# nomic-ai/contrastors

Hardware: AMD Instinct MI355X
Metric: query-doc pairs/sec (whole node), nomic-bert-2048 seq128 global-batch 16384 (higher is better)
Workload: dtype bf16

## Files before the change

### contrastors_amd/_C.py

```python
from __future__ import annotations

import ctypes as C
import os
from pathlib import Path

_PKG = Path(__file__).resolve().parent
LIB_PATH = Path(os.environ.get("CONTRASTORS_HIP_LIB", _PKG / "lib" / "libcontrastors_hip.so"))

CX_OK = 0
_ERR = {-1: "CX_ERR_SHAPE", -2: "CX_ERR_ALIGN", -3: "CX_ERR_ARG", -4: "CX_ERR_LAUNCH"}

vp = C.c_void_p
i32 = C.c_int
i64 = C.c_long
f32 = C.c_float
u64 = C.c_ulonglong
u32 = C.c_uint


class CxLayerWeights(C.Structure):
    _fields_ = (
        [(n, vp) for n in ("Wqkv", "Wout", "Wfc1", "Wfc2", "WqkvT", "WoutT", "Wfc1T", "Wfc2T")]
        + [(n, vp) for n in ("bqkv", "bout", "bfc1", "bfc2")]
        + [(n, vp) for n in ("ln1_g", "ln1_b", "ln2_g", "ln2_b")]
# ... 41 lines not shown


class CxVitExt(C.Structure):
    _fields_ = [("rope_cos", vp), ("rope_sin", vp), ("n_rope", i32), ("n_prefix", i32), ("no_final_ln", i32),
                ("subln_eps", f32), ("sub_ln", C.POINTER(CxVitSubLN)), ("z", vp), ("zmean", vp), ("zrstd", vp),
                ("yg_wide", vp)]


_SIGS = {
    "cx_abi_version": (i32, []),
    "cx_build_info": (C.c_char_p, []),
    "cx_error_string": (C.c_char_p, [i32]),
    "cx_gemm_bf16_nt": (i32, [vp, vp, vp, vp, i32, i32, i32, i32, i32, i32, i32, i32, f32, vp]),
    "cx_gemm_bf16_nt_accum": (i32, [vp, vp, vp, vp, i64, i32, i32, i32, i32, i32, vp]),
    "cx_gemm_bf16_tn_accum": (i32, [vp, vp, vp, vp, i64, i32, i32, i32, i32, i32, vp]),
    "cx_prof_gemm_config": (i32, [i32, i32]),
    "cx_prof_gemm_collect": (i32, [C.POINTER(C.c_double), C.POINTER(C.c_double), C.POINTER(i64), C.POINTER(i64)]),
    "cx_calib_mfma_bf16": (i32, [vp, i32, i32, vp, vp, vp]),
    "cx_calib_copy": (i32, [vp, vp, i64, vp]),
    "cx_transpose_bf16": (i32, [vp, vp, i32, i32, i32, i32, i32, vp]),
    "cx_cast_f32_to_bf16": (i32, [vp, vp, i64, vp]),
    "cx_cast_transpose_f32_to_bf16": (i32, [vp, vp, i32, i32, vp]),
    "cx_cast_transpose_f32_to_bf16_batched": (i32, [vp, i32, i32, vp]),
    "cx_cast_bf16_to_f32": (i32, [vp, vp, i64, vp]),
    "cx_layernorm_fwd": (i32, [vp, vp, vp, vp, vp, vp, vp, vp, i32, i32, f32, vp]),
    "cx_layernorm_bwd": (i32, [vp, vp, vp, vp, vp, vp, vp, vp, vp, vp, vp, i64, i32, i32, vp]),
    "cx_layernorm_bwd_pooled": (i32, [vp, vp, vp, vp, i32, i32, i32, vp, vp, vp, vp, vp, vp, vp, vp, vp, i64, i32, i32, vp]),
    "cx_layernorm_bwd_colsum": (i32, [vp, vp, vp, vp, vp, vp, vp, vp, vp, vp, vp, vp, i64, i32, i32, vp]),
    "cx_dropout_add_layernorm_fwd": (i32, [vp, vp, vp, vp, vp, vp, vp, vp, i32, i32, f32, f32, C.c_ulonglong, C.c_ulonglong,
                                           C.c_uint, vp]),
# ... 126 lines not shown
}

_DEV_SIGS = {
    "cx_gemm_set_variant": (None, [i32]),
    "cx_gemm_get_variant": (i32, []),
    "cx_gemm_set_debug": (None, [i32]),
    "cx_gemm_set_trace": (None, [vp]),
    "cx_gemm_v6_ablate": (None, [i32]),
    "cx_gemm_v6_trace": (None, [vp]),
    "cx_gemm_v7_mode": (None, [i32]),
    "cx_gemm_v7_trace": (None, [vp]),
    "cx_gemm_v7_occupancy": (i32, []),
    "cx_gemm_v7_ablate": (None, [i32]),
    "cx_gemm_v7_flags": (None, [i32]),
    "cx_gemm_v7_period": (None, [i32]),
    "cx_gemm_set_glds": (None, [i32]),
    "cx_gemm_get_glds": (i32, []),
    "cx_attn_set_bwd_s128": (None, [i32]),
    "cx_attn_set_prio": (None, [i32]),
    "cx_attn_set_fwd_s128": (None, [i32]),
    "cx_attn_set_fwd_long": (None, [i32]),
    "cx_attn_set_bwd_long": (None, [i32]),
    "cx_probe_mfma_layout": (i32, [vp, vp]),
    "cx_probe_ds_read_tr16": (i32, [vp, vp, vp]),
    "cx_probe_mfma_rate": (i32, [vp, i32, i32, i32, vp, vp, vp]),
    "cx_attn_dropout_keep_mask": (i32, [vp, i32, i32, i32, f32, u64, u64, u32, vp]),
    "cx_probe_rmw": (i32, [vp, i64, i32, i32, i32, vp]),
    "cx_probe_mfma_rate16": (i32, [vp, i32, i32, i32, vp, vp, vp]),
    "cx_probe_dma_bw": (i32, [vp, i64, i64, i64, i32, i32, i32, i32, vp, vp]),
}
# ... 58 lines not shown
```

### contrastors_amd/csrc/engine.hip

```cpp
#include <hip/hip_runtime.h>
#include "../../include/contrastors_hip.h"
#include "ln_workspace.h"

namespace {

#define CX_TRY(expr)              \
    do {                          \
        int rc__ = (expr);        \
        if (rc__ != CX_OK) return rc__; \
    } while (0)

inline long round_up(long v, long m) { return (v + m - 1) / m * m; }

inline int mark_grads_done(const CxChunkBuffers* buf, int idx, void* stream) {
    if (!buf->layer_events || !buf->layer_events[idx]) return CX_OK;
    return hipEventRecord((hipEvent_t)buf->layer_events[idx], (hipStream_t)stream) == hipSuccess ? CX_OK : CX_ERR_LAUNCH;
}

struct Slots {
    const CxChunkBuffers* b;
    const CxEncoderDesc* e;
    long T_cap;
    int d, I, wfc1;
    int mode;
// ... 58 lines not shown
    return (int)s;
}

int wgrad(const uint16_t* dY, int out_f, const uint16_t* X, int in_f, float* gW, const CxChunkBuffers* b, int T,
          void* stream) {
    if (!gW) return CX_OK;
    const int rc = cx_gemm_bf16_tn_accum(dY, X, gW, b->ws_f32, b->ws_floats, T, out_f, in_f, out_f, in_f, stream);
    if (rc != CX_ERR_SHAPE) return rc;
    if (!b->tr_a || !b->tr_b) return CX_ERR_ARG;
    const int Tp = (int)round_up(T, 64);
    CX_TRY(cx_transpose_bf16(dY, b->tr_a, T, out_f, out_f, Tp, Tp, stream));
    CX_TRY(cx_transpose_bf16(X, b->tr_b, T, in_f, in_f, Tp, Tp, stream));
    return cx_gemm_bf16_nt_accum(b->tr_a, b->tr_b, gW, b->ws_f32, b->ws_floats, out_f, in_f, Tp, Tp, Tp, stream);
}

int proj_residual(const uint16_t* x, const uint16_t* W, const float* bias, const uint16_t* residual, uint16_t* out, int T,
                  int N, int K, bool* folded, void* stream, const CxChunkBuffers* buf = nullptr) {
    *folded = false;
    if (buf && buf->ws_f32 && (long)((T + 255) / 256) * ((N + 255) / 256) <= 64 && K >= 1536) {
        const int rc = cx_gemm_bf16_nt_splitk(x, W, out, bias, residual, buf->ws_f32, buf->ws_floats, T, N, K, K, K, N, N, stream);
        if (rc != CX_ERR_SHAPE) {
            *folded = residual != nullptr && rc == CX_OK;
            return rc;
        }
    }
    if (residual) {
        const int rc = cx_gemm_bf16_nt_residual(x, W, out, bias, residual, T, N, K, K, K, N, N, stream);
        if (rc != CX_ERR_SHAPE) {
            *folded = rc == CX_OK;
            return rc;
// ... 174 lines not shown
};

int blocks_backward(const CxEncoderDesc* enc, const CxChunkBuffers* buf, const Slots& s, const int32_t* cu_seqlens, int Bc,
                    int T, int max_seqlen, const PooledGrad* pg, const uint16_t** da_out, const uint16_t** db_out, void* stream,
                    const CxVitExt* ext = nullptr) {
    const int d = enc->d, I = enc->d_inner, H = enc->n_head, L = enc->n_layer;
    auto mlp_bwd = [&](const CxLayerWeights& w, int l, const uint16_t* dm, const uint16_t* mlp_in, const uint16_t* add,
                       bool* folded, bool bias_done) -> int {
        if (w.gbfc2 && !bias_done) CX_TRY(cx_bias_grad(dm, w.gbfc2, T, d, d, stream));
        if (ext_subln(ext)) {
            CX_TRY(wgrad(dm, d, s.ez(ext, l), I, w.gWfc2, buf, T, stream));
            CX_TRY(cx_gemm_bf16_nt(dm, w.Wfc2T, buf->g_act, nullptr, T, I, d, d, d, I, 0, 1, 1.f, stream));
            const CxVitSubLN& n = ext->sub_ln[l];
            CX_TRY(cx_swiglu_subln_bwd(buf->g_act, s.act(l), s.yg(l), s.ezmean(ext, l), s.ezrstd(ext, l), n.norm_g, buf->g_wide,
                                       n.gnorm_g, n.gnorm_b, w.gbfc1, buf->ws_f32, buf->ws_floats, T, I, stream));
            CX_TRY(wgrad(buf->g_wide, s.wfc1, mlp_in, d, w.gWfc1, buf, T, stream));
            return proj_residual(buf->g_wide, w.Wfc1T, nullptr, add, buf->g_b, T, d, s.wfc1, folded, stream, buf);
        }
        CX_TRY(wgrad(dm, d, s.act(l), I, w.gWfc2, buf, T, stream));
        int fused = CX_ERR_SHAPE;
        if (enc->gated)
            fused = cx_gemm_bf16_swiglu_bwd_gate(dm, w.Wfc2T, s.act(l), s.yg(l), buf->g_wide, T, I, d, d, d, I, s.wfc1, stream);
#ifndef CX_AB_R5_ROUTES
        if (!enc->gated && gelu_fused_shape(T, s.wfc1, d))
            fused = cx_gemm_bf16_act_bwd(dm, w.Wfc2T, s.yg(l), buf->g_wide, w.gbfc1, buf->ws_f32, buf->ws_floats, T, I, d, d, d, I, I,
                                         enc->mlp_act, stream);
#endif
        if (fused != CX_ERR_SHAPE) {
            CX_TRY(fused);
        } else {
            CX_TRY(cx_gemm_bf16_nt(dm, w.Wfc2T, buf->g_act, nullptr, T, I, d, d, d, I, 0, 1, 1.f, stream));
        }
        if (enc->gated) {
            if (fused == CX_ERR_SHAPE)
                CX_TRY(cx_swiglu_bwd_gate(buf->g_act, s.act(l), s.yg(l), buf->g_wide, T, I, stream));
        } else if (fused == CX_ERR_SHAPE) {
            CX_TRY(cx_bias_act_bwd_colsum(buf->g_act, s.yg(l), gelu_fused_shape(T, s.wfc1, d) ? nullptr : w.bfc1, buf->g_wide,
                                          w.gbfc1, T, I, enc->mlp_act, stream));
        }
        CX_TRY(wgrad(buf->g_wide, s.wfc1, mlp_in, d, w.gWfc1, buf, T, stream));
        return proj_residual(buf->g_wide, w.Wfc1T, nullptr, add, buf->g_b, T, d, s.wfc1, folded, stream, buf);
    };
    auto attn_bwd = [&](const CxLayerWeights& w, int l, const uint16_t* dx, const uint16_t* attn_in, const uint16_t* add,
                        bool* folded, bool bias_done) -> int {
        if (w.gbout && !bias_done) CX_TRY(cx_bias_grad(dx, w.gbout, T, d, d, stream));
        CX_TRY(wgrad(dx, d, s.ctx(l), d, w.gWout, buf, T, stream));
        CX_TRY(cx_gemm_bf16_nt(dx, w.WoutT, buf->g_b, nullptr, T, d, d, d, d, d, 0, 1, 1.f, stream));
        if (buf->drop_active && enc->attn_pdrop > 0.f) {
            CX_TRY(cx_attn_varlen_dropout_bwd(buf->g_b, s.qkv(l), s.ctx(l), s.lse(l), cu_seqlens, enc->rot_cos, enc->rot_sin,
                                              buf->delta, buf->g_wide, Bc, H, T, max_seqlen, enc->softmax_scale, enc->attn_pdrop,
                                              buf->drop_seed, buf->drop_offset, (unsigned)(2 * enc->n_layer + 1 + l), stream));
        } else if (enc->rot_cos && max_seqlen > 128) {
            CX_TRY(cx_attn_varlen_bwd_prerotated(buf->g_b, s.qkv(l), s.ctx(l), s.lse(l), cu_seqlens, enc->rot_cos, enc->rot_sin,
                                                 buf->delta, buf->g_wide, Bc, H, T, max_seqlen, enc->softmax_scale, stream));
        } else {
            CX_TRY(cx_attn_varlen_bwd(buf->g_b, s.qkv(l), s.ctx(l), s.lse(l), cu_seqlens, enc->rot_cos, enc->rot_sin,
                                      buf->delta, buf->g_wide, Bc, H, T, max_seqlen, enc->softmax_scale, stream));
        }
        if (ext_rope(ext))
            CX_TRY(cx_rope2d_qkv_inplace(buf->g_wide, cu_seqlens, ext->rope_cos, ext->rope_sin, ext->n_rope, Bc, H, T, ext->n_prefix,
                                         -1, stream));
        if (w.gbqkv) CX_TRY(cx_bias_grad(buf->g_wide, w.gbqkv, T, 3 * d, 3 * d, stream));
        CX_TRY(wgrad(buf->g_wide, 3 * d, attn_in, d, w.gWqkv, buf, T, stream));
        return proj_residual(buf->g_wide, w.WqkvT, nullptr, add, buf->g_b, T, d, 3 * d, folded, stream, buf);
    };
    const bool ws_holds_colsum = cx_ln_bwd_ws_holds(buf->ws_f32, buf->ws_floats, 3, d);
    auto ln_bwd = [&](const uint16_t* a, const uint16_t* b2, const uint16_t* z, const float* g, const float* mean,
                      const float* rstd, const uint16_t* dz_extra, uint16_t* dz, float* gg, float* gb, float* gbias,
                      bool* done) -> int {
        *done = gbias && ws_holds_colsum;
        return cx_layernorm_bwd_colsum(a, b2, z, g, mean, rstd, dz_extra, dz, gg, gb, *done ? gbias : nullptr, buf->ws_f32,
                                       buf->ws_floats, T, d, stream);
    };
    const BlockRunner run{enc, buf, s, cu_seqlens, Bc, T, max_seqlen, stream, ext};
    if (!enc->prenorm) {
        const uint16_t* da = buf->g_a;
        const uint16_t* db = nullptr;
        for (int l = L - 1; l >= 0; --l) {
// ... 398 lines not shown

int cx_abi_version(void) { return 10; }
const char* cx_build_info(void) { return "contrastors_hip gfx950 " __DATE__ " " __VERSION__; }
const char* cx_error_string(int code) {
    switch (code) {
        case CX_OK: return "ok";
        case CX_ERR_SHAPE: return "unsupported shape";
        case CX_ERR_ALIGN: return "misaligned pointer or leading dimension";
        case CX_ERR_ARG: return "invalid argument";
        case CX_ERR_LAUNCH: return "kernel launch failed";
        default: return "unknown error";
    }
}

}
```

### contrastors_amd/csrc/gemm_api.hip

```cpp
#include "cx_common.h"
#include "../../include/contrastors_hip.h"
#include "gemm_params.h"
#include <mutex>

namespace {

constexpr int BK = 64;

__global__ __launch_bounds__(256) void splitk_reduce_kernel(const float* __restrict__ part, float* __restrict__ out, long n4,
                                                            long slab, int splits) {
    const long stride = (long)gridDim.x * blockDim.x;
    for (long i = (long)blockIdx.x * blockDim.x + threadIdx.x; i < n4; i += stride) {
        float4 a = reinterpret_cast<const float4*>(out)[i];
        for (int s = 0; s < splits; ++s) {
            const float4 v = reinterpret_cast<const float4*>(part + s * slab)[i];
            a.x += v.x; a.y += v.y; a.z += v.z; a.w += v.w;
        }
        reinterpret_cast<float4*>(out)[i] = a;
    }
}

int reduce_slabs(const float* ws, float* out, long slab, int split, hipStream_t s) {
    const long n4 = slab / 4;
    long g = (n4 + 255) / 256;
// ... 112 lines not shown
    if (ws_floats < slab) return CX_ERR_SHAPE;
    const int Tp = (T + BK - 1) / BK * BK;
    GemmParams p = base_params(dY, A, ws, nullptr, O, I, Tp, ld_dy, ld_a, I);
    const long tiles = (long)(O / 256) * (I / 256), nk = Tp / BK;
    long max_split = nk / 4;
    if (max_split > ws_floats / slab) max_split = ws_floats / slab;
    if (max_split > 32) max_split = 32;
    p.split_k = (int)choose_split(tiles, max_split);
    {
        ProfScope prof(2.0 * (double)T * (double)O * (double)I, (hipStream_t)stream);
        if (cx_launch_gemm_v6_tn(p, (hipStream_t)stream) != hipSuccess) return CX_ERR_LAUNCH;
    }
    return reduce_slabs(ws, G, slab, p.split_k, (hipStream_t)stream);
}

int cx_gemm_bf16_swiglu(const uint16_t* X, const uint16_t* W, uint16_t* YG, uint16_t* Act, int M, int I, int K, int ldx,
                        int ldw, int ld_yg, int ld_act, void* stream) {
    if (M <= 0 || I <= 0) return CX_OK;
    if (K <= 0 || (K % BK) != 0 || (I % 32) != 0) return CX_ERR_SHAPE;
    if ((ldx % 8) != 0 || (ldw % 8) != 0 || (ld_yg % 4) != 0 || (ld_act % 4) != 0) return CX_ERR_ALIGN;
    if (!Act) return CX_ERR_ARG;
    GemmParams p = base_params(X, W, YG, nullptr, M, 2 * I, K, ldx, ldw, ld_yg);
    p.Out2 = Act; p.ldo2 = ld_act;
    ProfScope prof(2.0 * (double)M * (double)(2 * I) * (double)K, (hipStream_t)stream);
    const hipError_t e = ((ld_yg % 8) == 0 && (ld_act % 8) == 0)
                             ? cx_launch_gemm_v6(p, GEMM_EPI_SWIGLU, (hipStream_t)stream)
                             : cx_launch_gemm_v5(p, 0, GEMM_OUT_BF16, GEMM_EPI_SWIGLU, (hipStream_t)stream);
    return e == hipSuccess ? CX_OK : CX_ERR_LAUNCH;
}

// ... 118 lines not shown
```

### contrastors_amd/csrc/gemm_bf16.hip

```cpp
#include "cx_common.h"
#include "../../include/contrastors_hip.h"
#include "gemm_params.h"

namespace {

constexpr int BM = 128, BN = 128, BK = 64;
constexpr int TILE_BYTES = 128 * BK * 2;

typedef __attribute__((address_space(3))) void* lds_void_ptr;
typedef const __attribute__((address_space(1))) void* glb_void_ptr;

enum OutMode { OUT_BF16 = GEMM_OUT_BF16, OUT_F32 = GEMM_OUT_F32, OUT_F32_ATOMIC = GEMM_OUT_F32_ATOMIC };

struct StageRegs { uint4 r0, r1, r2, r3; };

CX_DEVICE uint4 stage_load(const bf16_t* __restrict__ base, int ld, int row0, int nrows, int k0, int tid, int p) {
    const int r = p * 32 + (tid >> 3);
    int gr = row0 + r;
    gr = gr < nrows ? gr : nrows - 1;
    return *reinterpret_cast<const uint4*>(base + (size_t)gr * ld + k0 + (tid & 7) * 8);
}

template <bool GLDS>
CX_DEVICE void stage_tile(const bf16_t* __restrict__ base, int ld, int row0, int nrows, int k0, char* lds_tile,
// ... 721 lines not shown
    if (use_v5) {
        if (cx_launch_gemm_v5(p, 1, GEMM_OUT_F32_PARTIAL, GEMM_EPI_NONE, (hipStream_t)stream) != hipSuccess) return CX_ERR_LAUNCH;
    } else {
        hipLaunchKernelGGL(gemm_bf16_tn_kernel, dim3((int)(tiles * split)), dim3(512), V2_NSTAGE * V2_STAGE,
                           (hipStream_t)stream, p);
    }
    if (slot >= 0) (void)hipEventRecord(g_prof.ev1[slot], (hipStream_t)stream);
    if (hipGetLastError() != hipSuccess) return CX_ERR_LAUNCH;
    const long n4 = slab / 4;
    long g = (n4 + 255) / 256;
    if (g > 2048) g = 2048;
    hipLaunchKernelGGL(splitk_reduce_kernel, dim3((int)g), dim3(256), 0, (hipStream_t)stream, ws, G, n4, slab, (int)split);
    return hipGetLastError() == hipSuccess ? CX_OK : CX_ERR_LAUNCH;
}

int cx_gemm_bf16_swiglu(const uint16_t* X, const uint16_t* W, uint16_t* YG, uint16_t* Act, int M, int I, int K, int ldx,
                        int ldw, int ld_yg, int ld_act, void* stream) {
    if (M <= 0 || I <= 0) return CX_OK;
    if (K <= 0 || (K % BK) != 0 || (I % 32) != 0) return CX_ERR_SHAPE;
    if ((ldx % 8) != 0 || (ldw % 8) != 0 || (ld_yg % 4) != 0 || (ld_act % 4) != 0) return CX_ERR_ALIGN;
    if (!Act) return CX_ERR_ARG;
    GemmParams p;
    p.X = X; p.W = W; p.Out = YG; p.bias = nullptr;
    p.M = M; p.N = 2 * I; p.K = K; p.ldx = ldx; p.ldw = ldw; p.ldo = ld_yg;
    p.tiles_m = p.tiles_n = 0; p.split_k = 1; p.alpha = 1.f; p.dbg = g_dbg;
    p.Out2 = Act; p.ldo2 = ld_act; p.sup_m = p.sup_n = 0;
    int slot = -1;
    if (g_prof.enabled) {
        if ((g_prof.launches % g_prof.stride) == 0 && g_prof.used < GemmProf::CAP) {
            slot = g_prof.used++;
// ... 192 lines not shown
```

### contrastors_amd/csrc/gemm_bf16_v6.hip

```cpp
#include "cx_common.h"
#include "../../include/contrastors_hip.h"
#include "gemm_params.h"
#include <type_traits>

namespace {

#ifndef CX_V6_HI_EARLY
#define CX_V6_HI_EARLY 1
#endif
#ifndef CX_V6_OPAQUE
#define CX_V6_OPAQUE 1
#endif
#ifndef CX_V6_NT
#define CX_V6_NT 3
#endif
template <int J>
__device__ __forceinline__ void v6_dma_m0(uint32_t slot_base) {
    asm volatile("s_add_u32 m0, %0, %1" ::"s"(slot_base), "n"(J * 4096) : "memory", "scc");
}
__device__ __forceinline__ void v6_dma_ld(uint32_t off, const bf16_t* base) {
    asm volatile("global_load_lds_dwordx4 %0, %1" ::"v"(off), "s"(base) : "memory");
}
template <int J>
__device__ __forceinline__ void v6_dma_full(uint32_t slot_base, uint32_t off, const bf16_t* base) {
// ... 1117 lines not shown
template <int EPI, int DBG = 0>
hipError_t launch6(const GemmParams& p, hipStream_t stream) {
    static CxLdsOptIn lds;
    if (!lds.ensure(reinterpret_cast<const void*>(&gemm_bf16_v6_kernel<EPI, DBG>), LDS6)) return hipErrorInvalidValue;
    const int ntiles = p.tiles_m * p.tiles_n;
    const int grid = ntiles < 256 ? (ntiles + 7) / 8 * 8 : 256;
    hipLaunchKernelGGL((gemm_bf16_v6_kernel<EPI, DBG>), dim3(grid), dim3(256), LDS6, stream, p);
    return hipGetLastError();
}

typedef __attribute__((address_space(3))) bf16x4_t* lds_b4_ptr6;
constexpr int TNROW6 = 512;

CX_DEVICE int tn_swz(int t) { return ((t & 3) << 2) ^ (((t >> 3) & 1) << 1); }

__global__ __launch_bounds__(256, 1) __attribute__((amdgpu_waves_per_eu(1, 1))) void gemm_bf16_v6tn_kernel(GemmParams p) {
    extern __shared__ __attribute__((aligned(16))) char dsm[];
    const int tid = threadIdx.x;
    const int lane = tid & 63;
    const int wave = __builtin_amdgcn_readfirstlane(tid >> 6);
    const int l15 = lane & 15, g4 = lane >> 4;
    const int wm = wave >> 1, wn = wave & 1;
    const int nwg = p.tiles_m * p.tiles_n * p.split_k;
    int lid = xcd_remap(blockIdx.x, nwg);
    int tm, tn;
    if (p.tiles_m < p.tiles_n) {
        tm = lid % p.tiles_m;
        lid /= p.tiles_m;
        tn = lid % p.tiles_n;
        lid /= p.tiles_n;
    } else {
        tn = lid % p.tiles_n;
        lid /= p.tiles_n;
        tm = lid % p.tiles_m;
        lid /= p.tiles_m;
    }
    const int sk = lid;
    const int m0 = tm * BM6, n0 = tn * BN6;
    const int nk_total = p.K / BK6;
    const int kt_begin = (int)(((long)nk_total * sk) / p.split_k);
    const int kt_end = (int)(((long)nk_total * (sk + 1)) / p.split_k);
    const int nk = kt_end - kt_begin;
    if (nk <= 0) return;

    uint32_t xo[8], wo[8];
#pragma unroll
    for (int j = 0; j < 8; ++j) {
        const int t = (j * 4 + wave) * 2 + (lane >> 5);
        const int c = (lane & 31) ^ tn_swz(t);
        xo[j] = (uint32_t)t * (uint32_t)p.ldx * 2u + c * 16;
        wo[j] = (uint32_t)t * (uint32_t)p.ldw * 2u + c * 16;
    }
    const bf16_t* xb = p.X + (size_t)kt_begin * BK6 * p.ldx + m0;
    const bf16_t* wb = p.W + (size_t)kt_begin * BK6 * p.ldw + n0;
    const size_t xstep = (size_t)BK6 * p.ldx, wstep = (size_t)BK6 * p.ldw;
    int lx_slot = 0, lw_slot = 0;
    const uint32_t lds0 = (uint32_t)(uintptr_t)(lds_void_ptr)dsm;
    const uint32_t lds_wave = lds0 + wave * 1024;
    uint32_t x_m0 = lds_wave, w_m0 = lds_wave + 3 * XS6;
    auto issue_x_tile = [&]() {
        v6_dma_full<0>(x_m0, xo[0], xb); v6_dma_full<1>(x_m0, xo[1], xb); v6_dma_full<2>(x_m0, xo[2], xb); v6_dma_full<3>(x_m0, xo[3], xb);
        v6_dma_full<4>(x_m0, xo[4], xb); v6_dma_full<5>(x_m0, xo[5], xb); v6_dma_full<6>(x_m0, xo[6], xb); v6_dma_full<7>(x_m0, xo[7], xb);
    };
    auto issue_w_tile = [&]() {
        v6_dma_full<0>(w_m0, wo[0], wb); v6_dma_full<1>(w_m0, wo[1], wb); v6_dma_full<2>(w_m0, wo[2], wb); v6_dma_full<3>(w_m0, wo[3], wb);
        v6_dma_full<4>(w_m0, wo[4], wb); v6_dma_full<5>(w_m0, wo[5], wb); v6_dma_full<6>(w_m0, wo[6], wb); v6_dma_full<7>(w_m0, wo[7], wb);
    };
    auto x_advance = [&](int next) {
        xb += next < nk ? xstep : 0;
        lx_slot = lx_slot == 2 ? 0 : lx_slot + 1;
// ... 67 lines not shown
        asm volatile("s_waitcnt vmcnt(4)" ::: "memory");
        __builtin_amdgcn_s_barrier();
        CX_SEG(mma1, F1, 32, 64, F0, nxs_slot, nws_slot, 0, RS_ == 2 ? 32 : 33, RS_, 2, RS_ == 2 ? 33 : 49, RS_ == 2 ? 8 : DS_, 4, 4);
        x_advance(t + 3);
        xs_slot = nxs_slot;
        ws_slot = nws_slot;
    };
    kt_body(std::true_type{}, 0);
#pragma unroll 1
    for (int t = 1; t < nk; ++t) kt_body(std::false_type{}, t);
#undef CX_SEG
#undef CX_DMA_M0
#undef CX_DMA_LD

    asm volatile("s_waitcnt vmcnt(0)\n\ts_nop 7\n\ts_nop 7\n\ts_nop 7" ::: "memory");
    float* part = reinterpret_cast<float*>(p.Out) + (size_t)sk * p.M * p.ldo;
#pragma unroll
    for (int b = 0; b < 4; ++b) {
        float* rowp = part + (size_t)(m0 + wm * 128 + b * 32 + l15) * p.ldo + n0 + wn * 128 + 4 * g4;
        float* rowq = rowp + (size_t)16 * p.ldo;
#pragma unroll
        for (int a = 0; a < 4; ++a) v6_store_block_f32(4 * b + a, rowp + a * 32, rowq + a * 32);
    }
}

#ifndef CX_V7_POLICY
#define CX_V7_POLICY 1
#endif
#ifndef CX_PRODUCT
int g_v7_mode = -1;
#else
constexpr int g_v7_mode = -1;
#endif
bool v7_takes(const GemmParams& p, int epi) {
    const int mode = g_v7_mode >= 0 ? (g_v7_mode ? 2 : 0) : CX_V7_POLICY;
    if (mode == 0 || !cx_gemm_v7_covers(p, epi)) return false;
    if (mode == 2) return true;
// ... 31 lines not shown

#ifndef CX_PRODUCT
void cx_gemm_v6_set_trace(long long* buf) { g_v6_trace = buf; }
void cx_gemm_v6_set_ablate(int mask) { g_v6_dbg = mask; }
void cx_gemm_v6_force_groups(int gn) { g_v6_force_gn = (gn == 1 || gn == 2 || gn == 4 || gn == 8) ? gn : 0; }
void cx_gemm_v7_set_mode(int mode) { g_v7_mode = mode < 0 ? -1 : (mode ? 1 : 0); }
#endif

hipError_t cx_launch_gemm_v6_tn(GemmParams p, hipStream_t stream) {
    static CxLdsOptIn lds;
    if (!lds.ensure(reinterpret_cast<const void*>(&gemm_bf16_v6tn_kernel), LDS6)) return hipErrorInvalidValue;
    p.tiles_m = p.M / BM6;
    p.tiles_n = p.N / BN6;
    hipLaunchKernelGGL(gemm_bf16_v6tn_kernel, dim3(p.tiles_m * p.tiles_n * p.split_k), dim3(256), LDS6, stream, p);
    return hipGetLastError();
}

namespace {
__global__ __launch_bounds__(256) void colsum_part_reduce_kernel(const float* __restrict__ part, float* dst, int nblocks, int N) {
    __shared__ float red[4][64];
    const int col = blockIdx.x * 64 + (threadIdx.x & 63), grp = threadIdx.x >> 6;
    float sacc = 0.f;
    if (col < N) {
#pragma unroll 4
        for (int b = grp; b < nblocks; b += 4) sacc += part[(size_t)b * N + col];
    }
    red[grp][threadIdx.x & 63] = sacc;
    __syncthreads();
    if (grp == 0 && col < N) dst[col] += (red[0][threadIdx.x] + red[1][threadIdx.x]) + (red[2][threadIdx.x] + red[3][threadIdx.x]);
}
// ... 49 lines not shown
```

### contrastors_amd/csrc/gemm_params.h

```cpp
#pragma once
#include <hip/hip_runtime.h>
#include <stdint.h>

enum { GEMM_OUT_BF16 = 0, GEMM_OUT_F32 = 1, GEMM_OUT_F32_ATOMIC = 2, GEMM_OUT_F32_PARTIAL = 3 };
enum { GEMM_EPI_NONE = 0, GEMM_EPI_SWIGLU = 1, GEMM_EPI_GELU = 2, GEMM_EPI_SWIGLU_BWD = 3,
       GEMM_EPI_QGELU = 4,
       GEMM_EPI_SWIGLU_G = 5,
       GEMM_EPI_SWIGLU_BWD_AG = 6,
       GEMM_EPI_QACT_BWD = 8,
       GEMM_EPI_ACT_BWD = 7 };

struct GemmParams {
    const uint16_t* X;
    const uint16_t* W;
    void* Out;
    const float* bias;
    int M, N, K;
    int ldx, ldw, ldo;
    int tiles_m, tiles_n, split_k;
    float alpha;
    int dbg;
    int act;
    void* Out2;
    int ldo2;
    const uint16_t* In3;
    float* colsum_part;
    int sup_m, sup_n;
    long long* trace;
};

hipError_t cx_launch_gemm_v5(GemmParams p, int form, int out_mode, int epi, hipStream_t stream);
hipError_t cx_launch_gemm_v6(GemmParams p, int epi, hipStream_t stream);
void cx_gemm_v6_force_groups(int gn);
void cx_gemm_v6_set_trace(long long* buf);
void cx_gemm_v6_set_ablate(int mask);
hipError_t cx_launch_gemm_v6_tn(GemmParams p, hipStream_t stream);
hipError_t cx_launch_colsum_part_reduce(const float* part, float* dst, int nblocks, int N, hipStream_t stream);
bool cx_gemm_v7_covers(const GemmParams& p, int epi);
hipError_t cx_launch_gemm_v7(GemmParams p, int epi, int force_gn, hipStream_t stream);
void cx_gemm_v7_set_trace(long long* buf);
int cx_gemm_v7_occupancy_query(void);
void cx_gemm_v7_set_ablate(int mask);
void cx_gemm_v7_set_flags(int f);
void cx_gemm_v7_set_period(int cycles);
void cx_gemm_v7_set_mode(int mode);
void cx_gemm_v5_set_persistent(bool on);
void cx_gemm_v5_set_use_v6(bool on);
bool cx_gemm_v5_get_use_v6(void);
void cx_gemm_v5_set_trace(long long* buf);
```

### include/contrastors_hip.h

```cpp
#ifndef CONTRASTORS_HIP_H
#define CONTRASTORS_HIP_H

#include <stdint.h>

#ifdef __cplusplus
extern "C" {
#endif

#define CX_OK 0
#define CX_ERR_SHAPE (-1)
#define CX_ERR_ALIGN (-2)
#define CX_ERR_ARG (-3)
#define CX_ERR_LAUNCH (-4)

int cx_abi_version(void);
const char* cx_build_info(void);
const char* cx_error_string(int code);

int cx_gemm_bf16_nt(const uint16_t* X, const uint16_t* W, void* Out, const float* bias, int M, int N, int K, int ldx,
                    int ldw, int ldo, int out_mode, int split_k, float alpha, void* stream);
int cx_gemm_bf16_nt_accum(const uint16_t* X, const uint16_t* W, float* Out, float* ws, long ws_floats, int M, int N,
                          int K, int ldx, int ldw, void* stream);
int cx_gemm_bf16_tn_accum(const uint16_t* dY, const uint16_t* A, float* G, float* ws, long ws_floats, int T, int O, int I,
                          int ld_dy, int ld_a, void* stream);
int cx_prof_gemm_config(int enable, int stride);
int cx_prof_gemm_collect(double* total_ms, double* total_flop, long* launches_timed, long* launches_total);
int cx_calib_mfma_bf16(const void* seed_1024x16B, int iters, int nwg, long long* cycles_nwg_x4, float* sink, void* stream);
int cx_calib_copy(const void* src, void* dst, long bytes, void* stream);

int cx_transpose_bf16(const uint16_t* In, uint16_t* Out, int rows, int cols, int ld_in, int ld_out, int rows_pad,
                      void* stream);
int cx_cast_f32_to_bf16(const float* In, uint16_t* Out, long n, void* stream);
int cx_cast_transpose_f32_to_bf16(const float* In, uint16_t* OutT, int rows, int cols, void* stream);
typedef struct {
    const float* in;
    uint16_t* out_t;
    int rows, cols;
} CxCastJob;
int cx_cast_transpose_f32_to_bf16_batched(const CxCastJob* jobs, int n_jobs, int max_tiles, void* stream);
// ... 407 lines not shown
```

### include/contrastors_hip_dev.h

```cpp
#ifndef CONTRASTORS_HIP_DEV_H
#define CONTRASTORS_HIP_DEV_H

#include "contrastors_hip.h"

#ifdef __cplusplus
extern "C" {
#endif

void cx_gemm_set_variant(int v);
int cx_gemm_get_variant(void);

void cx_gemm_set_debug(int bits);

void cx_gemm_set_trace(void* buf);

void cx_gemm_v6_ablate(int mask);
void cx_gemm_v6_trace(void* buf);

void cx_gemm_v7_mode(int mode);
void cx_gemm_v7_trace(void* buf);
int cx_gemm_v7_occupancy(void);
void cx_gemm_v7_ablate(int mask);
void cx_gemm_v7_flags(int flags);
void cx_gemm_v7_period(int cycles);

void cx_gemm_set_glds(int enable);
int cx_gemm_get_glds(void);

void cx_attn_set_fwd_s128(int mode);
void cx_attn_set_bwd_s128(int mode);
void cx_attn_set_fwd_long(int on);
void cx_attn_set_bwd_long(int on);
void cx_attn_set_prio(int on);

int cx_probe_mfma_layout(float* out_32x32, void* stream);
int cx_probe_ds_read_tr16(const uint16_t* in_64x4, uint16_t* out_64x4, void* stream);
int cx_attn_dropout_keep_mask(unsigned char* keep, int B, int H, int S, float p_drop, unsigned long long seed,
                              unsigned long long offset, unsigned int site, void* stream);
int cx_probe_rmw(float* buf, long floats_per_problem, int sweeps, int n_problems, int nwg, void* stream);
int cx_probe_mfma_rate16(const void* seed_2048x16B, int waves, int iters, int nwg, long long* cycles_nwg_x8, float* sink,
// ... 11 lines not shown
```

Baseline: 4335.

## Group QKV and out-proj weight-gradient GEMMs into one persistent split-K launch

Adds a grouped TN weight-gradient GEMM that runs two problems (Wqkv and Wout grads) in a single persistent launch, using a static plan that splits K into slices. It also assigns the tail K-range to thin workgroups so the 256-WG grid stays evenly loaded, followed by one fused slab reduction. The FC1 weight gradient is routed through the same grouped kernel when it tiles evenly. This targets wave quantization and tail idle time from small-tile-count wgrad launches, as well as per-launch overhead. In exchange it adds a dependence on workspace size and a more complex reduction, and the Wout wgrad now runs later than before.

```diff
diff --git a/contrastors_amd/_C.py b/contrastors_amd/_C.py
--- a/contrastors_amd/_C.py
+++ b/contrastors_amd/_C.py
@@ -79,6 +79,8 @@
     "cx_gemm_bf16_nt": (i32, [vp, vp, vp, vp, i32, i32, i32, i32, i32, i32, i32, i32, f32, vp]),
     "cx_gemm_bf16_nt_accum": (i32, [vp, vp, vp, vp, i64, i32, i32, i32, i32, i32, vp]),
     "cx_gemm_bf16_tn_accum": (i32, [vp, vp, vp, vp, i64, i32, i32, i32, i32, i32, vp]),
+    "cx_gemm_bf16_tn_accum_grouped": (i32, [vp, vp, vp, i32, i32, i32, i32, vp, vp, vp, i32, i32, i32, i32, vp, i64, i32, vp]),
+    "cx_gemm_tn_plan": (i32, [i32, i32, i32, i32, i32, i64, C.POINTER(i32), C.POINTER(i32), i32]),
     "cx_prof_gemm_config": (i32, [i32, i32]),
     "cx_prof_gemm_collect": (i32, [C.POINTER(C.c_double), C.POINTER(C.c_double), C.POINTER(i64), C.POINTER(i64)]),
     "cx_calib_mfma_bf16": (i32, [vp, i32, i32, vp, vp, vp]),
@@ -235,6 +237,7 @@
     "cx_gemm_v7_ablate": (None, [i32]),
     "cx_gemm_v7_flags": (None, [i32]),
     "cx_gemm_v7_period": (None, [i32]),
+    "cx_engine_wgrad_grouping": (None, [i32]),
     "cx_gemm_set_glds": (None, [i32]),
     "cx_gemm_get_glds": (i32, []),
     "cx_attn_set_bwd_s128": (None, [i32]),
diff --git a/contrastors_amd/csrc/engine.hip b/contrastors_amd/csrc/engine.hip
--- a/contrastors_amd/csrc/engine.hip
+++ b/contrastors_amd/csrc/engine.hip
@@ -96,6 +96,35 @@
     return cx_gemm_bf16_nt_accum(b->tr_a, b->tr_b, gW, b->ws_f32, b->ws_floats, out_f, in_f, Tp, Tp, Tp, stream);
 }
 
+#ifndef CX_WGRAD_GROUPING
+#define CX_WGRAD_GROUPING 1
+#endif
+#ifndef CX_PRODUCT
+int g_wgrad_grouping = CX_WGRAD_GROUPING;
+#else
+constexpr int g_wgrad_grouping = CX_WGRAD_GROUPING;
+#endif
+
+int wgrad_pair(const uint16_t* dYa, int out_a, const uint16_t* Xa, int in_a, float* gWa, const uint16_t* dYb, int out_b,
+               const uint16_t* Xb, int in_b, float* gWb, const CxChunkBuffers* b, int T, void* stream) {
+    if (g_wgrad_grouping && gWa && gWb) {
+        const int rc = cx_gemm_bf16_tn_accum_grouped(dYa, Xa, gWa, out_a, in_a, out_a, in_a, dYb, Xb, gWb, out_b, in_b, out_b,
+                                                     in_b, b->ws_f32, b->ws_floats, T, stream);
+        if (rc != CX_ERR_SHAPE) return rc;
+    }
+    CX_TRY(wgrad(dYb, out_b, Xb, in_b, gWb, b, T, stream));
+    return wgrad(dYa, out_a, Xa, in_a, gWa, b, T, stream);
+}
+
+int wgrad_even(const uint16_t* dY, int out_f, const uint16_t* X, int in_f, float* gW, const CxChunkBuffers* b, int T, void* stream) {
+    if (g_wgrad_grouping && gW && (out_f % 256) == 0 && (in_f % 256) == 0 && (long)(out_f / 256) * (in_f / 256) >= 64) {
+        const int rc = cx_gemm_bf16_tn_accum_grouped(dY, X, gW, out_f, in_f, out_f, in_f, nullptr, nullptr, nullptr, 0, 0, 0, 0,
+                                                     b->ws_f32, b->ws_floats, T, stream);
+        if (rc != CX_ERR_SHAPE) return rc;
+    }
+    return wgrad(dY, out_f, X, in_f, gW, b, T, stream);
+}
+
 int proj_residual(const uint16_t* x, const uint16_t* W, const float* bias, const uint16_t* residual, uint16_t* out, int T,
                   int N, int K, bool* folded, void* stream, const CxChunkBuffers* buf = nullptr) {
     *folded = false;
@@ -300,7 +329,7 @@
             const CxVitSubLN& n = ext->sub_ln[l];
             CX_TRY(cx_swiglu_subln_bwd(buf->g_act, s.act(l), s.yg(l), s.ezmean(ext, l), s.ezrstd(ext, l), n.norm_g, buf->g_wide,
                                        n.gnorm_g, n.gnorm_b, w.gbfc1, buf->ws_f32, buf->ws_floats, T, I, stream));
-            CX_TRY(wgrad(buf->g_wide, s.wfc1, mlp_in, d, w.gWfc1, buf, T, stream));
+            CX_TRY(wgrad_even(buf->g_wide, s.wfc1, mlp_in, d, w.gWfc1, buf, T, stream));
             return proj_residual(buf->g_wide, w.Wfc1T, nullptr, add, buf->g_b, T, d, s.wfc1, folded, stream, buf);
         }
         CX_TRY(wgrad(dm, d, s.act(l), I, w.gWfc2, buf, T, stream));
@@ -324,13 +353,12 @@
             CX_TRY(cx_bias_act_bwd_colsum(buf->g_act, s.yg(l), gelu_fused_shape(T, s.wfc1, d) ? nullptr : w.bfc1, buf->g_wide,
                                           w.gbfc1, T, I, enc->mlp_act, stream));
         }
-        CX_TRY(wgrad(buf->g_wide, s.wfc1, mlp_in, d, w.gWfc1, buf, T, stream));
+        CX_TRY(wgrad_even(buf->g_wide, s.wfc1, mlp_in, d, w.gWfc1, buf, T, stream));
         return proj_residual(buf->g_wide, w.Wfc1T, nullptr, add, buf->g_b, T, d, s.wfc1, folded, stream, buf);
     };
     auto attn_bwd = [&](const CxLayerWeights& w, int l, const uint16_t* dx, const uint16_t* attn_in, const uint16_t* add,
                         bool* folded, bool bias_done) -> int {
         if (w.gbout && !bias_done) CX_TRY(cx_bias_grad(dx, w.gbout, T, d, d, stream));
-        CX_TRY(wgrad(dx, d, s.ctx(l), d, w.gWout, buf, T, stream));
         CX_TRY(cx_gemm_bf16_nt(dx, w.WoutT, buf->g_b, nullptr, T, d, d, d, d, d, 0, 1, 1.f, stream));
         if (buf->drop_active && enc->attn_pdrop > 0.f) {
             CX_TRY(cx_attn_varlen_dropout_bwd(buf->g_b, s.qkv(l), s.ctx(l), s.lse(l), cu_seqlens, enc->rot_cos, enc->rot_sin,
@@ -347,7 +375,7 @@
             CX_TRY(cx_rope2d_qkv_inplace(buf->g_wide, cu_seqlens, ext->rope_cos, ext->rope_sin, ext->n_rope, Bc, H, T, ext->n_prefix,
                                          -1, stream));
         if (w.gbqkv) CX_TRY(cx_bias_grad(buf->g_wide, w.gbqkv, T, 3 * d, 3 * d, stream));
-        CX_TRY(wgrad(buf->g_wide, 3 * d, attn_in, d, w.gWqkv, buf, T, stream));
+        CX_TRY(wgrad_pair(buf->g_wide, 3 * d, attn_in, d, w.gWqkv, dx, d, s.ctx(l), d, w.gWout, buf, T, stream));
         return proj_residual(buf->g_wide, w.WqkvT, nullptr, add, buf->g_b, T, d, 3 * d, folded, stream, buf);
     };
     const bool ws_holds_colsum = cx_ln_bwd_ws_holds(buf->ws_f32, buf->ws_floats, 3, d);
@@ -776,3 +804,7 @@
 }
 
 }
+
+#ifndef CX_PRODUCT
+extern "C" void cx_engine_wgrad_grouping(int on) { g_wgrad_grouping = on != 0; }
+#endif
diff --git a/contrastors_amd/csrc/gemm_api.hip b/contrastors_amd/csrc/gemm_api.hip
--- a/contrastors_amd/csrc/gemm_api.hip
+++ b/contrastors_amd/csrc/gemm_api.hip
@@ -150,6 +150,21 @@
     return reduce_slabs(ws, G, slab, p.split_k, (hipStream_t)stream);
 }
 
+int cx_gemm_bf16_tn_accum_grouped(const uint16_t* dY0, const uint16_t* A0, float* G0, int O0, int I0, int ld_dy0, int ld_a0,
+                                  const uint16_t* dY1, const uint16_t* A1, float* G1, int O1, int I1, int ld_dy1, int ld_a1,
+                                  float* ws, long ws_floats, int T, void* stream) {
+    if (T <= 0) return CX_OK;
+    const TnGroupedArgs a = {{dY0, dY1}, {A0, A1}, {G0, G1}, {O0, O1}, {I0, I1}, {ld_dy0, ld_dy1}, {ld_a0, ld_a1}, ws, ws_floats, T};
+    CxTnPlan plan;
+    const int rc = cx_tn_grouped_plan(a, plan);
+    if (rc != CX_OK) return rc;
+    {
+        ProfScope prof(2.0 * (double)T * ((double)O0 * I0 + (G1 ? (double)O1 * I1 : 0.0)), (hipStream_t)stream);
+        if (cx_launch_gemm_v6_tn_grouped(a, plan, (hipStream_t)stream) != hipSuccess) return CX_ERR_LAUNCH;
+    }
+    return cx_launch_tn_grouped_reduce(a, plan, (hipStream_t)stream) == hipSuccess ? CX_OK : CX_ERR_LAUNCH;
+}
+
 int cx_gemm_bf16_swiglu(const uint16_t* X, const uint16_t* W, uint16_t* YG, uint16_t* Act, int M, int I, int K, int ldx,
                         int ldw, int ld_yg, int ld_act, void* stream) {
     if (M <= 0 || I <= 0) return CX_OK;
diff --git a/contrastors_amd/csrc/gemm_bf16.hip b/contrastors_amd/csrc/gemm_bf16.hip
--- a/contrastors_amd/csrc/gemm_bf16.hip
+++ b/contrastors_amd/csrc/gemm_bf16.hip
@@ -759,6 +759,18 @@
     return hipGetLastError() == hipSuccess ? CX_OK : CX_ERR_LAUNCH;
 }
 
+int cx_gemm_bf16_tn_accum_grouped(const uint16_t* dY0, const uint16_t* A0, float* G0, int O0, int I0, int ld_dy0, int ld_a0,
+                                  const uint16_t* dY1, const uint16_t* A1, float* G1, int O1, int I1, int ld_dy1, int ld_a1,
+                                  float* ws, long ws_floats, int T, void* stream) {
+    if (T <= 0) return CX_OK;
+    const TnGroupedArgs a = {{dY0, dY1}, {A0, A1}, {G0, G1}, {O0, O1}, {I0, I1}, {ld_dy0, ld_dy1}, {ld_a0, ld_a1}, ws, ws_floats, T};
+    CxTnPlan plan;
+    const int rc = cx_tn_grouped_plan(a, plan);
+    if (rc != CX_OK) return rc;
+    if (cx_launch_gemm_v6_tn_grouped(a, plan, (hipStream_t)stream) != hipSuccess) return CX_ERR_LAUNCH;
+    return cx_launch_tn_grouped_reduce(a, plan, (hipStream_t)stream) == hipSuccess ? CX_OK : CX_ERR_LAUNCH;
+}
+
 int cx_gemm_bf16_swiglu(const uint16_t* X, const uint16_t* W, uint16_t* YG, uint16_t* Act, int M, int I, int K, int ldx,
                         int ldw, int ld_yg, int ld_act, void* stream) {
     if (M <= 0 || I <= 0) return CX_OK;
diff --git a/contrastors_amd/csrc/gemm_bf16_v6.hip b/contrastors_amd/csrc/gemm_bf16_v6.hip
--- a/contrastors_amd/csrc/gemm_bf16_v6.hip
+++ b/contrastors_amd/csrc/gemm_bf16_v6.hip
@@ -1155,46 +1155,26 @@
 
 CX_DEVICE int tn_swz(int t) { return ((t & 3) << 2) ^ (((t >> 3) & 1) << 1); }
 
-__global__ __launch_bounds__(256, 1) __attribute__((amdgpu_waves_per_eu(1, 1))) void gemm_bf16_v6tn_kernel(GemmParams p) {
+CX_DEVICE void v6tn_unit(const bf16_t* X, const bf16_t* W, int ldx, int ldw, int m0, int n0, int kt_begin, int nk, float* part,
+                         int ldo) {
     extern __shared__ __attribute__((aligned(16))) char dsm[];
     const int tid = threadIdx.x;
     const int lane = tid & 63;
     const int wave = __builtin_amdgcn_readfirstlane(tid >> 6);
     const int l15 = lane & 15, g4 = lane >> 4;
     const int wm = wave >> 1, wn = wave & 1;
-    const int nwg = p.tiles_m * p.tiles_n * p.split_k;
-    int lid = xcd_remap(blockIdx.x, nwg);
-    int tm, tn;
-    if (p.tiles_m < p.tiles_n) {
-        tm = lid % p.tiles_m;
-        lid /= p.tiles_m;
-        tn = lid % p.tiles_n;
-        lid /= p.tiles_n;
-    } else {
-        tn = lid % p.tiles_n;
-        lid /= p.tiles_n;
-        tm = lid % p.tiles_m;
-        lid /= p.tiles_m;
-    }
-    const int sk = lid;
-    const int m0 = tm * BM6, n0 = tn * BN6;
-    const int nk_total = p.K / BK6;
-    const int kt_begin = (int)(((long)nk_total * sk) / p.split_k);
-    const int kt_end = (int)(((long)nk_total * (sk + 1)) / p.split_k);
-    const int nk = kt_end - kt_begin;
-    if (nk <= 0) return;
 
     uint32_t xo[8], wo[8];
 #pragma unroll
     for (int j = 0; j < 8; ++j) {
         const int t = (j * 4 + wave) * 2 + (lane >> 5);
         const int c = (lane & 31) ^ tn_swz(t);
-        xo[j] = (uint32_t)t * (uint32_t)p.ldx * 2u + c * 16;
-        wo[j] = (uint32_t)t * (uint32_t)p.ldw * 2u + c * 16;
-    }
-    const bf16_t* xb = p.X + (size_t)kt_begin * BK6 * p.ldx + m0;
-    const bf16_t* wb = p.W + (size_t)kt_begin * BK6 * p.ldw + n0;
-    const size_t xstep = (size_t)BK6 * p.ldx, wstep = (size_t)BK6 * p.ldw;
+        xo[j] = (uint32_t)t * (uint32_t)ldx * 2u + c * 16;
+        wo[j] = (uint32_t)t * (uint32_t)ldw * 2u + c * 16;
+    }
+    const bf16_t* xb = X + (size_t)kt_begin * BK6 * ldx + m0;
+    const bf16_t* wb = W + (size_t)kt_begin * BK6 * ldw + n0;
+    const size_t xstep = (size_t)BK6 * ldx, wstep = (size_t)BK6 * ldw;
     int lx_slot = 0, lw_slot = 0;
     const uint32_t lds0 = (uint32_t)(uintptr_t)(lds_void_ptr)dsm;
     const uint32_t lds_wave = lds0 + wave * 1024;
@@ -1292,13 +1272,80 @@
 #undef CX_DMA_LD
 
     asm volatile("s_waitcnt vmcnt(0)\n\ts_nop 7\n\ts_nop 7\n\ts_nop 7" ::: "memory");
-    float* part = reinterpret_cast<float*>(p.Out) + (size_t)sk * p.M * p.ldo;
 #pragma unroll
     for (int b = 0; b < 4; ++b) {
-        float* rowp = part + (size_t)(m0 + wm * 128 + b * 32 + l15) * p.ldo + n0 + wn * 128 + 4 * g4;
-        float* rowq = rowp + (size_t)16 * p.ldo;
+        float* rowp = part + (size_t)(m0 + wm * 128 + b * 32 + l15) * ldo + n0 + wn * 128 + 4 * g4;
+        float* rowq = rowp + (size_t)16 * ldo;
 #pragma unroll
         for (int a = 0; a < 4; ++a) v6_store_block_f32(4 * b + a, rowp + a * 32, rowq + a * 32);
+    }
+}
+
+__global__ __launch_bounds__(256, 1) __attribute__((amdgpu_waves_per_eu(1, 1))) void gemm_bf16_v6tn_kernel(GemmParams p) {
+    const int nwg = p.tiles_m * p.tiles_n * p.split_k;
+    int lid = xcd_remap(blockIdx.x, nwg);
+    int tm, tn;
+    if (p.tiles_m < p.tiles_n) {
+        tm = lid % p.tiles_m;
+        lid /= p.tiles_m;
+        tn = lid % p.tiles_n;
+        lid /= p.tiles_n;
+    } else {
+        tn = lid % p.tiles_n;
+        lid /= p.tiles_n;
+        tm = lid % p.tiles_m;
+        lid /= p.tiles_m;
+    }
+    const int sk = lid;
+    const int nk_total = p.K / BK6;
+    const int kt_begin = (int)(((long)nk_total * sk) / p.split_k);
+    const int kt_end = (int)(((long)nk_total * (sk + 1)) / p.split_k);
+    if (kt_end <= kt_begin) return;
+    v6tn_unit(p.X, p.W, p.ldx, p.ldw, tm * BM6, tn * BN6, kt_begin, kt_end - kt_begin,
+              reinterpret_cast<float*>(p.Out) + (size_t)sk * p.M * p.ldo, p.ldo);
+}
+
+struct GemmTnGroup {
+    const bf16_t* X0; const bf16_t* W0; float* part0;
+    const bf16_t* X1; const bf16_t* W1; float* part1;
+    int ldx0, ldw0, M0, N0;
+    int ldx1, ldw1, M1, N1;
+    CxTnPlan plan;
+};
+
+__global__ __launch_bounds__(256, 1) __attribute__((amdgpu_waves_per_eu(1, 1))) void gemm_bf16_v6tn_grouped_kernel(GemmTnGroup g) {
+    const int lid = xcd_remap(blockIdx.x, gridDim.x);
+    const int nu = cx_tn_unit_count(g.plan, lid);
+#pragma unroll 1
+    for (int i = 0; i < nu; ++i) {
+        const CxTnUnit u = cx_tn_unit(g.plan, lid, i);
+        const bool second = u.prob != 0;
+        const int M = second ? g.M1 : g.M0, N = second ? g.N1 : g.N0;
+        float* part = (second ? g.part1 : g.part0) + (size_t)u.slab * M * N;
+        v6tn_unit(second ? g.X1 : g.X0, second ? g.W1 : g.W0, second ? g.ldx1 : g.ldx0, second ? g.ldw1 : g.ldw0, u.tm * BM6,
+                  u.tn * BN6, u.kt_begin, u.kt_end - u.kt_begin, part, N);
+        asm volatile("s_waitcnt vmcnt(0) lgkmcnt(0)" ::: "memory");
+        __builtin_amdgcn_s_barrier();
+    }
+}
+
+__global__ __launch_bounds__(256) void tn_grouped_reduce_kernel(const float* __restrict__ part0, float* __restrict__ G0, long n4_0,
+                                                                const float* __restrict__ part1, float* __restrict__ G1, long n4_1,
+                                                                int nslab) {
+    const long stride = (long)gridDim.x * blockDim.x;
+    for (long i = (long)blockIdx.x * blockDim.x + threadIdx.x; i < n4_0 + n4_1; i += stride) {
+        const bool second = i >= n4_0;
+        const long n4 = second ? n4_1 : n4_0, e = second ? i - n4_0 : i;
+        const float4* part = reinterpret_cast<const float4*>(second ? part1 : part0);
+        float4 a = part[e];
+        for (int s = 1; s < nslab; ++s) {
+            const float4 v = part[s * n4 + e];
+            a.x += v.x; a.y += v.y; a.z += v.z; a.w += v.w;
+        }
+        float4* out = reinterpret_cast<float4*>(second ? G1 : G0) + e;
+        float4 o = *out;
+        o.x += a.x; o.y += a.y; o.z += a.z; o.w += a.w;
+        *out = o;
     }
 }
 
@@ -1360,6 +1407,59 @@
     p.tiles_n = p.N / BN6;
     hipLaunchKernelGGL(gemm_bf16_v6tn_kernel, dim3(p.tiles_m * p.tiles_n * p.split_k), dim3(256), LDS6, stream, p);
     return hipGetLastError();
+}
+
+int cx_tn_grouped_plan(const TnGroupedArgs& a, CxTnPlan& plan) {
+    const bool two = a.G[1] != nullptr;
+    if (a.O[0] <= 0 || a.I[0] <= 0 || (a.O[0] % 256) != 0 || (a.I[0] % 256) != 0) return CX_ERR_SHAPE;
+    if (two && (a.O[1] <= 0 || a.I[1] <= 0 || (a.O[1] % 256) != 0 || (a.I[1] % 256) != 0)) return CX_ERR_SHAPE;
+    if ((a.ld_dy[0] % 8) != 0 || (a.ld_a[0] % 8) != 0 || (two && ((a.ld_dy[1] % 8) != 0 || (a.ld_a[1] % 8) != 0))) return CX_ERR_ALIGN;
+    if (!a.ws || !a.G[0] || !a.dY[0] || !a.A[0] || (two && (!a.dY[1] || !a.A[1]))) return CX_ERR_ARG;
+    return cx_tn_make_plan(plan, a.T, a.O[0], a.I[0], two ? a.O[1] : 0, two ? a.I[1] : 0, a.ws_floats) ? CX_OK : CX_ERR_SHAPE;
+}
+
+hipError_t cx_launch_gemm_v6_tn_grouped(const TnGroupedArgs& a, const CxTnPlan& plan, hipStream_t stream) {
+    static CxLdsOptIn lds;
+    if (!lds.ensure(reinterpret_cast<const void*>(&gemm_bf16_v6tn_grouped_kernel), LDS6)) return hipErrorInvalidValue;
+    GemmTnGroup g = {};
+    g.X0 = a.dY[0]; g.W0 = a.A[0]; g.part0 = a.ws;
+    g.ldx0 = a.ld_dy[0]; g.ldw0 = a.ld_a[0]; g.M0 = a.O[0]; g.N0 = a.I[0];
+    if (plan.n > plan.n0) {
+        g.X1 = a.dY[1]; g.W1 = a.A[1]; g.part1 = a.ws + (size_t)plan.nslab * a.O[0] * a.I[0];
+        g.ldx1 = a.ld_dy[1]; g.ldw1 = a.ld_a[1]; g.M1 = a.O[1]; g.N1 = a.I[1];
+    }
+    g.plan = plan;
+    hipLaunchKernelGGL(gemm_bf16_v6tn_grouped_kernel, dim3(cx_tn_grid(plan)), dim3(256), LDS6, stream, g);
+    return hipGetLastError();
+}
+
+hipError_t cx_launch_tn_grouped_reduce(const TnGroupedArgs& a, const CxTnPlan& plan, hipStream_t stream) {
+    const bool two = plan.n > plan.n0;
+    const long n4_0 = (long)a.O[0] * a.I[0] / 4, n4_1 = two ? (long)a.O[1] * a.I[1] / 4 : 0;
+    long grid = (n4_0 + n4_1 + 255) / 256;
+    if (grid > 2048) grid = 2048;
+    hipLaunchKernelGGL(tn_grouped_reduce_kernel, dim3((int)grid), dim3(256), 0, stream, a.ws, a.G[0], n4_0,
+                       a.ws + (size_t)plan.nslab * a.O[0] * a.I[0], two ? a.G[1] : nullptr, n4_1, plan.nslab);
+    return hipGetLastError();
+}
+
+extern "C" int cx_gemm_tn_plan(int T, int O0, int I0, int O1, int I1, long ws_floats, int* plan_out, int* units, int max_units) {
+    CxTnPlan P;
+    if (!cx_tn_make_plan(P, T, O0, I0, O1, I1, ws_floats)) return CX_ERR_SHAPE;
+    if (plan_out) {
+        const int v[8] = {cx_tn_grid(P), P.nslab, P.S, P.nkb, P.nk, P.thin_wgs, P.q, P.n};
+        for (int i = 0; i < 8; ++i) plan_out[i] = v[i];
+    }
+    int count = 0;
+    for (int lid = 0; lid < cx_tn_grid(P); ++lid) {
+        for (int i = 0; i < cx_tn_unit_count(P, lid); ++i, ++count) {
+            if (!units || count >= max_units) continue;
+            const CxTnUnit u = cx_tn_unit(P, lid, i);
+            const int v[7] = {lid, u.prob, u.tm, u.tn, u.kt_begin, u.kt_end, u.slab};
+            for (int k = 0; k < 7; ++k) units[7 * count + k] = v[k];
+        }
+    }
+    return count;
 }
 
 namespace {
diff --git a/contrastors_amd/csrc/gemm_params.h b/contrastors_amd/csrc/gemm_params.h
--- a/contrastors_amd/csrc/gemm_params.h
+++ b/contrastors_amd/csrc/gemm_params.h
@@ -1,6 +1,7 @@
 #pragma once
 #include <hip/hip_runtime.h>
 #include <stdint.h>
+#include "gemm_tn_plan.h"
 
 enum { GEMM_OUT_BF16 = 0, GEMM_OUT_F32 = 1, GEMM_OUT_F32_ATOMIC = 2, GEMM_OUT_F32_PARTIAL = 3 };
 enum { GEMM_EPI_NONE = 0, GEMM_EPI_SWIGLU = 1, GEMM_EPI_GELU = 2, GEMM_EPI_SWIGLU_BWD = 3,
@@ -35,6 +36,18 @@
 void cx_gemm_v6_set_trace(long long* buf);
 void cx_gemm_v6_set_ablate(int mask);
 hipError_t cx_launch_gemm_v6_tn(GemmParams p, hipStream_t stream);
+struct TnGroupedArgs {
+    const uint16_t* dY[2];
+    const uint16_t* A[2];
+    float* G[2];
+    int O[2], I[2], ld_dy[2], ld_a[2];
+    float* ws;
+    long ws_floats;
+    int T;
+};
+int cx_tn_grouped_plan(const TnGroupedArgs& a, CxTnPlan& plan);
+hipError_t cx_launch_gemm_v6_tn_grouped(const TnGroupedArgs& a, const CxTnPlan& plan, hipStream_t stream);
+hipError_t cx_launch_tn_grouped_reduce(const TnGroupedArgs& a, const CxTnPlan& plan, hipStream_t stream);
 hipError_t cx_launch_colsum_part_reduce(const float* part, float* dst, int nblocks, int N, hipStream_t stream);
 bool cx_gemm_v7_covers(const GemmParams& p, int epi);
 hipError_t cx_launch_gemm_v7(GemmParams p, int epi, int force_gn, hipStream_t stream);
diff --git a/contrastors_amd/csrc/gemm_tn_plan.h b/contrastors_amd/csrc/gemm_tn_plan.h
--- /dev/null
+++ b/contrastors_amd/csrc/gemm_tn_plan.h
@@ -0,0 +1,98 @@
+#pragma once
+
+#ifdef __HIPCC__
+#define CX_TN_HD __host__ __device__ inline
+#else
+#define CX_TN_HD inline
+#endif
+
+#ifndef CX_TN_UNIT_COST
+#define CX_TN_UNIT_COST 16
+#endif
+enum { CX_TN_WGS = 256, CX_TN_MAX_SLICES = 32 };
+
+struct CxTnPlan {
+    int tiles_m[2], tiles_n[2];
+    int n0, n;
+    int nk;
+    int S, nkb;
+    int thin_wgs, q;
+    int bulk_wgs;
+    int nslab;
+};
+
+struct CxTnUnit {
+    int prob, tm, tn;
+    int kt_begin, kt_end;
+    int slab;
+};
+
+inline bool cx_tn_make_plan(CxTnPlan& P, int T, int O0, int I0, int O1, int I1, long ws_floats) {
+    if (T <= 0 || O0 <= 0 || I0 <= 0 || (O0 % 256) != 0 || (I0 % 256) != 0 || O1 < 0 || I1 < 0 || (O1 % 256) != 0 || (I1 % 256) != 0)
+        return false;
+    P = CxTnPlan{};
+    P.tiles_m[0] = O0 / 256; P.tiles_n[0] = I0 / 256;
+    P.tiles_m[1] = (O1 && I1) ? O1 / 256 : 0; P.tiles_n[1] = (O1 && I1) ? I1 / 256 : 0;
+    P.n0 = P.tiles_m[0] * P.tiles_n[0];
+    P.n = P.n0 + P.tiles_m[1] * P.tiles_n[1];
+    P.nk = (T + 63) / 64;
+    const long slabs = (long)P.n * 65536;
+    if (ws_floats < slabs) return false;
+    const int fill = CX_TN_WGS / P.n;
+    long S = fill < 1 ? 1 : fill;
+    if (S > P.nk / 4) S = P.nk / 4 < 1 ? 1 : P.nk / 4;
+    if (S > CX_TN_MAX_SLICES) S = CX_TN_MAX_SLICES;
+    if (S > ws_floats / slabs) S = ws_floats / slabs;
+    P.S = (int)S;
+    P.nkb = P.nk;
+    const int R = CX_TN_WGS - P.n * P.S;
+    if (P.S == fill && R > 0 && R < P.n && (S + 1) * slabs <= ws_floats) {
+        const int q = (P.n + R - 1) / R, c = CX_TN_UNIT_COST;
+        const int num = P.nk - P.S * c * (q - 1);
+        const int kr = num > 0 ? num / (P.S * q + 1) : 0;
+        if (kr >= 1) {
+            P.q = q;
+            P.thin_wgs = (P.n + q - 1) / q;
+            P.nkb = P.nk - kr;
+        }
+    }
+    const long bulk = (long)P.n * P.S;
+    P.bulk_wgs = bulk < CX_TN_WGS ? (int)bulk : CX_TN_WGS;
+    P.nslab = P.S + (P.thin_wgs ? 1 : 0);
+    return true;
+}
+
+CX_TN_HD int cx_tn_grid(const CxTnPlan& P) { return P.bulk_wgs + P.thin_wgs; }
+
+CX_TN_HD int cx_tn_unit_count(const CxTnPlan& P, int lid) {
+    if (lid < P.bulk_wgs) return (P.n * P.S - lid + P.bulk_wgs - 1) / P.bulk_wgs;
+    return (P.n - (lid - P.bulk_wgs) + P.thin_wgs - 1) / P.thin_wgs;
+}
+
+CX_TN_HD CxTnUnit cx_tn_unit(const CxTnPlan& P, int lid, int i) {
+    CxTnUnit u;
+    int t;
+    if (lid < P.bulk_wgs) {
+        const int id = lid + i * P.bulk_wgs, s = id / P.n;
+        t = id - s * P.n;
+        u.kt_begin = (int)(((long)P.nkb * s) / P.S);
+        u.kt_end = (int)(((long)P.nkb * (s + 1)) / P.S);
+        u.slab = s;
+    } else {
+        t = (lid - P.bulk_wgs) + i * P.thin_wgs;
+        u.kt_begin = P.nkb;
+        u.kt_end = P.nk;
+        u.slab = P.S;
+    }
+    u.prob = t >= P.n0 ? 1 : 0;
+    if (u.prob) t -= P.n0;
+    const int tms = P.tiles_m[u.prob], tns = P.tiles_n[u.prob];
+    if (tms < tns) {
+        u.tm = t % tms;
+        u.tn = t / tms;
+    } else {
+        u.tn = t % tns;
+        u.tm = t / tns;
+    }
+    return u;
+}
diff --git a/include/contrastors_hip.h b/include/contrastors_hip.h
--- a/include/contrastors_hip.h
+++ b/include/contrastors_hip.h
@@ -23,6 +23,10 @@
                           int K, int ldx, int ldw, void* stream);
 int cx_gemm_bf16_tn_accum(const uint16_t* dY, const uint16_t* A, float* G, float* ws, long ws_floats, int T, int O, int I,
                           int ld_dy, int ld_a, void* stream);
+int cx_gemm_bf16_tn_accum_grouped(const uint16_t* dY0, const uint16_t* A0, float* G0, int O0, int I0, int ld_dy0, int ld_a0,
+                                  const uint16_t* dY1, const uint16_t* A1, float* G1, int O1, int I1, int ld_dy1, int ld_a1,
+                                  float* ws, long ws_floats, int T, void* stream);
+int cx_gemm_tn_plan(int T, int O0, int I0, int O1, int I1, long ws_floats, int* plan_out, int* units, int max_units);
 int cx_prof_gemm_config(int enable, int stride);
 int cx_prof_gemm_collect(double* total_ms, double* total_flop, long* launches_timed, long* launches_total);
 int cx_calib_mfma_bf16(const void* seed_1024x16B, int iters, int nwg, long long* cycles_nwg_x4, float* sink, void* stream);
diff --git a/include/contrastors_hip_dev.h b/include/contrastors_hip_dev.h
--- a/include/contrastors_hip_dev.h
+++ b/include/contrastors_hip_dev.h
@@ -24,6 +24,8 @@
 void cx_gemm_v7_flags(int flags);
 void cx_gemm_v7_period(int cycles);
 
+void cx_engine_wgrad_grouping(int on);
+
 void cx_gemm_set_glds(int enable);
 int cx_gemm_get_glds(void);
 
```

Result: no change. 4338, median of 6 (+0.1%).
